# tobwei/APTAI

Measured on AMD Instinct MI355X. Metric: utterances/sec (10 s @ 16 kHz) train-step, higher is better.
Workload: dtype bf16

## Files before the change

### aptai_amd/_lib.py

```python
from __future__ import annotations

import ctypes
import os
import subprocess
import threading

import torch

_HERE = os.path.dirname(os.path.abspath(__file__))
CSRC = os.path.join(_HERE, "csrc")
LIB_PATH = os.environ.get("APTAI_HIP_LIB") or os.path.join(CSRC, "libaptai_hip.so")

_lib = None
_lock = threading.Lock()

_P, _I64, _I, _F, _U64 = ctypes.c_void_p, ctypes.c_int64, ctypes.c_int, ctypes.c_float, ctypes.c_uint64
ARGTYPES = {
    "aptai_layernorm_fwd": [_P, _P, _P, _P, _P, _P, _I64, _I64, _F, _I, _P],
    "aptai_layernorm_bwd": [_P, _P, _P, _P, _P, _P, _P, _P, _F, _U64, _P, _P, _P, _I64, _I64, _P, _P],
    "aptai_layernorm_bwd_workspace_bytes": [_I64, _I64],
    "aptai_layernorm_bwd_finalize_multi": [_P, _I64, _I64, _P],
    "aptai_layernorm_fwd_f32in": [_P, _P, _P, _P, _P, _I64, _I64, _F, _P],
    "aptai_layernorm_fwd_f32in_split": [_P, _P, _P, _P, _P, _I, _I64, _I64, _F, _P],
    "aptai_attention_fwd": [_P, _P, _P, _P, _P, _I64, _I64, _I64, _I64, _F, _F, _U64, _I, _P],
    "aptai_attention_bwd": [_P, _P, _P, _P, _P, _P, _P, _P, _I64, _I64, _I64, _I64, _F, _F, _U64, _I, _I, _P],
    "aptai_cast_f32_to_bf16": [_P, _P, _I64, _I64, _I64, _P],
    "aptai_conv_weight_to_bf16": [_P, _P, _I64, _I64, _I64, _P],
    "aptai_posconv_weight": [_P, _P, _P, _P, _P, _I64, _I64, _I64, _P],
    "aptai_posconv_pack": [_P, _P, _P, _P, _I64, _I64, _I64, _I64, _I64, _P],
    "aptai_frame_mask_fwd": [_P, _P, _P, _P, _I64, _I64, _I64, _I64, _P],
    "aptai_frame_mask_bwd": [_P, _P, _P, _P, _P, _I64, _I64, _I64, _I64, _P],
    "aptai_frame_mask_bwd_workspace_bytes": [_I64, _I64, _I64],
    "aptai_colsum_bf16": [_P, _I64, _P, _P, _I64, _I64, _I, _P],
    "aptai_colsum_workspace_bytes": [_I64, _I64],
    "aptai_dropout_bf16": [_P, _P, _I64, _F, _U64, _P],
    "aptai_dgelu_bf16": [_P, _P, _P, _I64, _P],
    "aptai_conv0_fwd": [_P, _I64, _I64, _P, _P, _P, _P, _I, _F, _P, _I64, _I64, _I64, _I64, _I64, _P, _P, _P],
    "aptai_conv0_bwd": [_P, _I64, _I64, _P, _P, _P, _P, _I, _F, _P, _I64, _I64, _P, _P, _P, _P, _P, _P, _P],
    "aptai_conv0_bwd_workspace_bytes": [_I64, _I64],
    "aptai_conv0_workspace_bytes": [_I64, _I64],
# ... 103 lines not shown
```

### aptai_amd/csrc/attention.hip

```cpp
#include "common.h"

namespace {

#ifdef APTAI_STAMPS
__device__ unsigned long long g_attn_stamps[3 * 1024 * 8];
#define ATTN_STAMP(k, slot)                                                                                       \
    do {                                                                                                          \
        if (threadIdx.x == 0) {                                                                                   \
            const int bl = blockIdx.x + gridDim.x * (blockIdx.y + gridDim.y * blockIdx.z);                        \
            if (bl < 1024) g_attn_stamps[((k) * 1024 + bl) * 8 + (slot)] = wall_clock64();                         \
        }                                                                                                         \
    } while (0)
#else
#define ATTN_STAMP(k, slot) do {} while (0)
#endif

constexpr int HD = 64;
constexpr float LOG2E = 1.4426950408889634f;

struct AttnArgs {
    const bf16_t* qkv; long ld;
    const int* lens;
    bf16_t* ctx; long ldo;
    float* lse2;
    float* o32;
    int B, Tp, H, heads;
    float c;
    float scale;
    uint32_t seed0, seed1, thr16; float dscale;
    const uint32_t* salt;
    const bf16_t* dctx;
    float* delta;
    bf16_t* dqkv;
    int skip_pad_q;
    int stagger;
    int xcd_remap;
    int q_prescaled;
};

__device__ __forceinline__ int tile_swz(int row) { return ((row >> 2) & 3) | (((row >> 1) & 1) << 2); }
__device__ __forceinline__ int tile_off(int row, int chunk) { return row * 128 + ((chunk ^ tile_swz(row)) << 4); }

struct LaneOffs {
    int rowk[4];
    int tr[2][2];
};
__device__ __forceinline__ LaneOffs lane_offs(int lane) {
    LaneOffs o;
    const int r31 = lane & 31, h = lane >> 5;
#pragma unroll
    for (int ds = 0; ds < 4; ++ds) o.rowk[ds] = tile_off(r31, 2 * ds + h);
    const int dgrp = (lane >> 4) & 1, i = lane & 15, qq = i >> 2, p = i & 3;
    const int trow = 4 * h + qq;
// ... 13 lines not shown
    return __builtin_bit_cast(bf16x8, r);
}

__device__ __forceinline__ bf16x8 pack8(const float* v) {
    u32x4 u = {pack2bf(v[0], v[1]), pack2bf(v[2], v[3]), pack2bf(v[4], v[5]), pack2bf(v[6], v[7])};
    return __builtin_bit_cast(bf16x8, u);
}

__device__ __forceinline__ int acc_row(int r, int h) { return (r & 3) + 8 * (r >> 2) + 4 * h; }

constexpr int OUT_PITCH = 144;
constexpr int STAGE_BYTES = 4 * 32 * OUT_PITCH;
constexpr int DQ_STAGE = 2 * 128 * 128;
constexpr int DKDV_BLOCKS = 3;
constexpr int DKDV_KV_BYTES = 2 * 128 * 128;

__device__ __forceinline__ void stage_rows128(char* dst, const bf16_t* src, long ld, int tid) {
#pragma unroll
    for (int it = 0; it < 4; ++it) {
        const int cid = it * 256 + tid, row = cid >> 3, ch = cid & 7;
        *(u32x4*)(dst + tile_off(row, ch)) = *(const u32x4*)(src + (long)row * ld + ch * 8);
    }
}
__device__ __forceinline__ void store_rows_bf16(char* sw, const f32x16 (&acc)[2], float scale, bf16_t* g_row0, long ld, int lane) {
    const int r31 = lane & 31, h = lane >> 5;
#pragma unroll
    for (int dt = 0; dt < 2; ++dt)
#pragma unroll
        for (int g4 = 0; g4 < 4; ++g4) {
            const int d = dt * 32 + 8 * g4 + 4 * h;
// ... 19 lines not shown
    int L = blockIdx.x + nt * (blockIdx.y + gridDim.y * blockIdx.z);
    if (a.xcd_remap && (total & 7) == 0) L = (L & 7) * (total >> 3) + (L >> 3);
    tile = L % nt;
    const int grp = L / nt;
    hd = grp % (int)gridDim.y;
    b = grp / (int)gridDim.y;
}

constexpr int FWD_BUF = 2 * 64 * 128;
constexpr int FWD_SMEM = 2 * FWD_BUF;
constexpr float REF_HEADROOM = 40.0f;
constexpr float REF_SUM_LIMIT = 1.4901161193847656e-08f;

template <bool V> struct Flag { static constexpr bool value = V; };

template <bool DROP>
__global__ __launch_bounds__(256, 3) void attn_fwd_kernel(AttnArgs a) {
    __shared__ __attribute__((aligned(16))) char smem[FWD_SMEM];
    ATTN_STAMP(0, 0);
    if (DROP) apply_salt(a.salt, a.seed0, a.seed1);
    const int tid = threadIdx.x, lane = tid & 63, wave = tid >> 6, h = lane >> 5;
    int tile_x, hd, b;
    attn_block(a, tile_x, hd, b);
    const int q0 = tile_x * 128 + wave * 32;
    int len = a.lens[b];
    len = len < 1 ? 1 : (len > a.Tp ? a.Tp : len);
    const int ntiles = (len + 63) >> 6;
    const long rowbase = (long)b * a.Tp;
    const int q = q0 + (lane & 31);
    const bf16_t* Qg = a.qkv + (rowbase + q) * a.ld + hd * HD;
    const bf16_t* Kg = a.qkv + rowbase * a.ld + a.H + hd * HD;
    const bf16_t* Vg = Kg + a.H;
// ... 11 lines not shown

    int soff[2];
    long goff[2];
#pragma unroll
    for (int it = 0; it < 2; ++it) {
        const int cid = it * 256 + tid, row = cid >> 3, ch = cid & 7;
        soff[it] = tile_off(row, ch);
        goff[it] = (long)row * a.ld + ch * 8;
    }
    u32x4 kreg[2], vreg[2];
    const long tile_stride = 64 * a.ld;
#pragma unroll
    for (int it = 0; it < 2; ++it) { kreg[it] = *(const u32x4*)(Kg + goff[it]); vreg[it] = *(const u32x4*)(Vg + goff[it]); }
    uint32_t hbase = 0;
    if (DROP) hbase = rng_hash((uint32_t)((b * a.heads + hd) * a.Tp + q), a.seed0, a.seed1) + (uint32_t)(2 * h) * ATTN_K1;
    const float c = a.c;
#pragma unroll
    for (int it = 0; it < 2; ++it) { *(u32x4*)(smem + soff[it]) = kreg[it]; *(u32x4*)(smem + 64 * 128 + soff[it]) = vreg[it]; }
    if (ntiles > 1) {
#pragma unroll
        for (int it = 0; it < 2; ++it) {
            kreg[it] = *(const u32x4*)(Kg + tile_stride + goff[it]);
            vreg[it] = *(const u32x4*)(Vg + tile_stride + goff[it]);
        }
    }
    __syncthreads();
    ATTN_STAMP(0, 1);

    auto tile = [&](auto first_flag, auto mask_flag, const int t) {
        constexpr bool FIRST = decltype(first_flag)::value, MASK = decltype(mask_flag)::value;
// ... 28 lines not shown
            for (int kt2 = 0; kt2 < 2; ++kt2)
#pragma unroll
                for (int r = 0; r < 16; ++r)
                    if (kbase + kt2 * 32 + acc_row(r, h) >= len) sT[kt2][r] = -INFINITY;
        }
        if (FIRST) {
            float mt = sT[0][0];
#pragma unroll
            for (int r = 1; r < 16; ++r) mt = fmaxf(mt, sT[0][r]);
#pragma unroll
            for (int r = 0; r < 16; ++r) mt = fmaxf(mt, sT[1][r]);
            mt = fmaxf(mt, __shfl_xor(mt, 32, 64));
            ref = fmaf(mt, c, REF_HEADROOM);
        }
        float psum = 0.f;
#pragma unroll
        for (int kt2 = 0; kt2 < 2; ++kt2) {
            bf16x8 vfr[2][2];
#pragma unroll
            for (int s = 0; s < 2; ++s)
#pragma unroll
                for (int dt = 0; dt < 2; ++dt) vfr[s][dt] = rd_tr(sV, lo, 2 * kt2 + s, dt);
            float x[16];
#pragma unroll
            for (int r = 0; r < 16; ++r) { x[r] = fast_exp2(fmaf(sT[kt2][r], c, -ref)); psum += x[r]; }
            if (DROP) {
#pragma unroll
                for (int r = 0; r < 16; r += 2) {
                    const uint32_t hsh = attn_mix(hbase + (uint32_t)(kbase / 2 + 16 * kt2 + acc_row(r, 0) / 2) * ATTN_K1);
                    x[r] = (hsh & 0xffffu) >= a.thr16 ? x[r] : 0.f;
                    x[r + 1] = (hsh >> 16) >= a.thr16 ? x[r + 1] : 0.f;
                }
            }
            const bf16x8 pf0 = pack8(&x[0]), pf1 = pack8(&x[8]);
#pragma unroll
            for (int dt = 0; dt < 2; ++dt) oT[dt] = __builtin_amdgcn_mfma_f32_32x32x16_bf16(vfr[0][dt], pf0, oT[dt], 0, 0, 0);
#pragma unroll
            for (int dt = 0; dt < 2; ++dt) oT[dt] = __builtin_amdgcn_mfma_f32_32x32x16_bf16(vfr[1][dt], pf1, oT[dt], 0, 0, 0);
        }
        psum += __shfl_xor(psum, 32, 64);
        l_run += psum;
        if (!FIRST && __builtin_amdgcn_ballot_w64(!(psum <= REF_SUM_LIMIT))) {
            if (!(psum <= REF_SUM_LIMIT)) {
                const float e = floorf(fast_log2(psum)) + REF_HEADROOM;
                const float sc = fast_exp2(-e);
                ref += e;
                l_run *= sc;
#pragma unroll
                for (int r = 0; r < 16; ++r) { oT[0][r] *= sc; oT[1][r] *= sc; }
            }
        }
        __syncthreads();
    };
    if (ntiles == 1) {
// ... 36 lines not shown
            __syncthreads();
#pragma unroll
            for (int i = 0; i < 4; ++i) {
                const int idx = i * 64 + lane, r = idx >> 3, ch = idx & 7;
                *(f32x4*)(a.o32 + orow + (long)r * a.ldo + dt * 32 + ch * 4) = *(const f32x4*)(sw + r * OUT_PITCH + ch * 16);
            }
        }
    }
    ATTN_STAMP(0, 3);
#ifdef APTAI_STAMPS
    asm volatile("s_waitcnt vmcnt(0)" ::: "memory");
    ATTN_STAMP(0, 4);
#endif
}

template <bool PRE>
__global__ __launch_bounds__(256, PRE ? DKDV_BLOCKS : 2) void attn_bwd_dkdv_kernel(AttnArgs a) {
    __shared__ __attribute__((aligned(16))) char smem[STAGE_BYTES + 384 + DKDV_KV_BYTES];
    char* sQ = smem;
    char* sD = smem + 32 * 128;
    float* sL = (float*)(smem + STAGE_BYTES);
    char* sKall = smem + STAGE_BYTES + 384;
    char* sVall = sKall + 128 * 128;
    ATTN_STAMP(1, 0);
    if (a.thr16) apply_salt(a.salt, a.seed0, a.seed1);
    const int tid = threadIdx.x, lane = tid & 63, wave = tid >> 6, h = lane >> 5;
    int tile_x, hd, b;
    attn_block(a, tile_x, hd, b);
    const int kb0 = tile_x * 128;
    const int key0 = kb0 + wave * 32;
    int len = a.lens[b];
    len = len < 1 ? 1 : (len > a.Tp ? a.Tp : len);
    const long rowbase = (long)b * a.Tp;
    const int key = key0 + (lane & 31);
    bf16_t* dK0 = a.dqkv + (rowbase + kb0) * a.ld + a.H + hd * HD;
    bf16_t* dV0 = dK0 + a.H;
    if (kb0 >= len) {
// ... 20 lines not shown
    const float* del = a.delta + ((long)b * a.heads + hd) * a.Tp;
    const int srow = tid >> 3, sch = tid & 7;
    const int soff = tile_off(srow, sch);
    const long gq = (long)srow * a.ld + sch * 8, gd = (long)srow * a.ldo + sch * 8;
    u32x4 qreg = *(const u32x4*)(Qb + gq), dreg = *(const u32x4*)(Db + gd);
    const float* stat = (tid < 8 ? lse : del) + (tid & 7) * 4;
    f32x4 sreg = (f32x4)(0.f);
    if (tid < 16) sreg = *(const f32x4*)stat;
    const bool key_ok = key < len;
    const bool wave_boundary = key0 + 32 > len;
    const uint32_t hshift = (key & 1) ? 16u : 0u;
    const float c = a.c;
    const uint32_t pairk = (uint32_t)(key >> 1) * ATTN_K1;
    const uint32_t rowid0 = (uint32_t)((b * a.heads + hd) * a.Tp) + (uint32_t)(tid & 31);
    uint32_t hreg = 0;
    if (a.thr16 && tid >= 32 && tid < 64) hreg = rng_hash(rowid0, a.seed0, a.seed1);
    ATTN_STAMP(1, 1);
    for (int t = 0; t < nq; ++t) {
        __syncthreads();
        *(u32x4*)(sQ + soff) = qreg;
        *(u32x4*)(sD + soff) = dreg;
        if (tid < 16) *(f32x4*)(sL + tid * 4) = PRE ? -sreg : sreg;
        if (a.thr16 && tid >= 32 && tid < 64) ((uint32_t*)sL)[64 + (tid & 31)] = hreg;
        __syncthreads();
        if (t + 1 < nq) {
            qreg = *(const u32x4*)(Qb + (long)(t + 1) * 32 * a.ld + gq);
            dreg = *(const u32x4*)(Db + (long)(t + 1) * 32 * a.ldo + gd);
            if (tid < 16) sreg = *(const f32x4*)(stat + (t + 1) * 32);
            if (a.thr16 && tid >= 32 && tid < 64) hreg = rng_hash(rowid0 + (uint32_t)((t + 1) * 32), a.seed0, a.seed1);
        }
        f32x16 cs = (f32x16)(0.f), cd = (f32x16)(0.f);
        if (PRE) {
#pragma unroll
            for (int g4 = 0; g4 < 4; ++g4) {
                const f32x4 l4 = *(const f32x4*)(sL + 8 * g4 + 4 * h);
                const f32x4 d4 = *(const f32x4*)(sL + 32 + 8 * g4 + 4 * h);
#pragma unroll
                for (int rr = 0; rr < 4; ++rr) { cs[4 * g4 + rr] = l4[rr]; cd[4 * g4 + rr] = d4[rr]; }
            }
        }
        f32x16 s = __builtin_amdgcn_mfma_f32_32x32x16_bf16(rd_row(sQ, lo, 0, 0), rd_row(sKall, lo, wave, 0), cs, 0, 0, 0);
        f32x16 dp = __builtin_amdgcn_mfma_f32_32x32x16_bf16(rd_row(sD, lo, 0, 0), rd_row(sVall, lo, wave, 0), cd, 0, 0, 0);
#pragma unroll
        for (int ds = 1; ds < 4; ++ds) {
// ... 11 lines not shown
                const f32x4 d4 = *(const f32x4*)(sL + 32 + 8 * g4 + 4 * h);
#pragma unroll
                for (int rr = 0; rr < 4; ++rr) {
                    pd[4 * g4 + rr] = fast_exp2(fmaf(s[4 * g4 + rr], c, -l4[rr]));
                    dsv[4 * g4 + rr] = d4[rr];
                }
            }
        }
        if (wave_boundary) {
#pragma unroll
            for (int r = 0; r < 16; ++r) pd[r] = key_ok ? pd[r] : 0.f;
        }
        if (a.thr16) {
#pragma unroll
            for (int g4 = 0; g4 < 4; ++g4) {
                const u32x4 rh = *(const u32x4*)((const uint32_t*)sL + 64 + 8 * g4 + 4 * h);
                f32x4 nd4 = (f32x4)(0.f);
                if (PRE) nd4 = *(const f32x4*)(sL + 32 + 8 * g4 + 4 * h);
#pragma unroll
                for (int rr = 0; rr < 4; ++rr) {
                    const int r = 4 * g4 + rr;
                    const uint32_t y = attn_mix(rh[rr] + pairk);
                    const bool k = ((y >> hshift) & 0xffffu) >= a.thr16;
                    const float p0 = pd[r];
                    if (PRE) dsv[r] = p0 * (k ? dp[r] : nd4[rr]);
                    else dsv[r] = p0 * ((k ? dp[r] : 0.f) - dsv[r]);
                    pd[r] = k ? p0 : 0.f;
                }
            }
        } else {
#pragma unroll
            for (int r = 0; r < 16; ++r) dsv[r] = PRE ? pd[r] * dp[r] : pd[r] * (dp[r] - dsv[r]);
        }
#pragma unroll
        for (int sstep = 0; sstep < 2; ++sstep) {
            const bf16x8 pf = pack8(&pd[8 * sstep]);
// ... 5 lines not shown
            }
        }
    }
    __syncthreads();
    ATTN_STAMP(1, 2);
    char* sw = smem + wave * (32 * OUT_PITCH);
    store_rows_bf16(sw, dKT, (PRE ? 0.6931471805599453f : a.scale) * a.dscale, dK0 + (long)(wave * 32) * a.ld, a.ld, lane);
    store_rows_bf16(sw, dVT, a.dscale, dV0 + (long)(wave * 32) * a.ld, a.ld, lane);
    ATTN_STAMP(1, 3);
#ifdef APTAI_STAMPS
    asm volatile("s_waitcnt vmcnt(0)" ::: "memory");
    ATTN_STAMP(1, 4);
#endif
}

template <bool PRE>
__global__ __launch_bounds__(256, 3) void attn_bwd_dq_kernel(AttnArgs a) {
    __shared__ __attribute__((aligned(16))) char smem[DQ_STAGE + 512];
    char* sK = smem;
    char* sV = smem + 32 * 128;
    float* sDel = (float*)(smem + DQ_STAGE);
    ATTN_STAMP(2, 0);
    if (a.thr16) apply_salt(a.salt, a.seed0, a.seed1);
    const int tid = threadIdx.x, lane = tid & 63, wave = tid >> 6, h = lane >> 5;
    int tile_x, hd, b;
    attn_block(a, tile_x, hd, b);
    const int qb0 = tile_x * 128;
    const int q = qb0 + wave * 32 + (lane & 31);
    int len = a.lens[b];
    len = len < 1 ? 1 : (len > a.Tp ? a.Tp : len);
    const long rowbase = (long)b * a.Tp;
// ... 53 lines not shown
        acc += __shfl_xor(acc, 4, 64);
        acc += __shfl_xor(acc, 2, 64);
        acc += __shfl_xor(acc, 1, 64);
        if (part == 0) sDel[row] = acc;
    }
    ATTN_STAMP(2, 7);
    __syncthreads();
    float del_q = sDel[wave * 32 + (lane & 31)];
    __syncthreads();
    del_q *= __frcp_rn(a.dscale);
    if (h == 0) a.delta[((long)b * a.heads + hd) * a.Tp + q] = del_q;
    f32x16 dQT[2];
    dQT[0] = dQT[1] = (f32x16)(0.f);
    const int nk = (len + 31) >> 5;
    uint32_t hbase = 0;
    if (a.thr16) hbase = rng_hash((uint32_t)((b * a.heads + hd) * a.Tp + q), a.seed0, a.seed1) + (uint32_t)(2 * h) * ATTN_K1;
    const float c = a.c;
    const f32x16 cs = (f32x16)(PRE ? -lse_q : 0.f), cd = (f32x16)(PRE ? -del_q : 0.f);
    ATTN_STAMP(2, 1);
    for (int t = 0; t < nk; ++t) {
        __syncthreads();
        *(u32x4*)(sK + soff) = kreg;
        *(u32x4*)(sV + soff) = vreg;
        __syncthreads();
        if (t + 1 < nk) {
            kreg = *(const u32x4*)(Kb + (long)(t + 1) * 32 * a.ld + gk);
            vreg = *(const u32x4*)(Vb + (long)(t + 1) * 32 * a.ld + gk);
        }
        f32x16 sT = __builtin_amdgcn_mfma_f32_32x32x16_bf16(rd_row(sK, lo, 0, 0), qf[0], cs, 0, 0, 0);
        f32x16 dpT = __builtin_amdgcn_mfma_f32_32x32x16_bf16(rd_row(sV, lo, 0, 0), df[0], cd, 0, 0, 0);
#pragma unroll
        for (int ds = 1; ds < 4; ++ds) {
            sT = __builtin_amdgcn_mfma_f32_32x32x16_bf16(rd_row(sK, lo, 0, ds), qf[ds], sT, 0, 0, 0);
            dpT = __builtin_amdgcn_mfma_f32_32x32x16_bf16(rd_row(sV, lo, 0, ds), df[ds], dpT, 0, 0, 0);
        }
        float dsv[16];
        const bool boundary = t * 32 + 32 > len;
#pragma unroll
        for (int r = 0; r < 16; ++r) {
            float p = PRE ? fast_exp2(sT[r]) : fast_exp2(fmaf(sT[r], c, -lse_q));
            if (boundary && (t * 32 + acc_row(r, h) >= len)) p = 0.f;
            dsv[r] = p;
        }
        if (a.thr16) {
            const float dropped = PRE ? -del_q : 0.f;
#pragma unroll
            for (int r = 0; r < 16; r += 2) {
                const uint32_t hsh = attn_mix(hbase + (uint32_t)(t * 16 + acc_row(r, 0) / 2) * ATTN_K1);
                dpT[r] = (hsh & 0xffffu) >= a.thr16 ? dpT[r] : dropped;
                dpT[r + 1] = (hsh >> 16) >= a.thr16 ? dpT[r + 1] : dropped;
            }
        }
#pragma unroll
        for (int r = 0; r < 16; ++r) dsv[r] *= PRE ? dpT[r] : (dpT[r] - del_q);
#pragma unroll
        for (int sstep = 0; sstep < 2; ++sstep) {
            const bf16x8 dsf = pack8(&dsv[8 * sstep]);
#pragma unroll
            for (int dt = 0; dt < 2; ++dt)
                dQT[dt] = __builtin_amdgcn_mfma_f32_32x32x16_bf16(rd_tr(sK, lo, sstep, dt), dsf, dQT[dt], 0, 0, 0);
        }
    }
    __syncthreads();
    ATTN_STAMP(2, 2);
    store_rows_bf16(smem + wave * (32 * OUT_PITCH), dQT, a.scale * a.dscale,
// ... 223 lines not shown
    static const int stagger = getenv("APTAI_ATTN_STAGGER") ? atoi(getenv("APTAI_ATTN_STAGGER")) : 0;
    a.stagger = stagger;
    static const int remap = getenv("APTAI_ATTN_XCD_REMAP") ? atoi(getenv("APTAI_ATTN_XCD_REMAP")) : 1;
    a.xcd_remap = remap;
    return APTAI_OK;
}

}

#ifdef APTAI_STAMPS
extern "C" int aptai_debug_read_attn_stamps(void* host_out) {
    return hipMemcpyFromSymbol(host_out, HIP_SYMBOL(g_attn_stamps), sizeof(g_attn_stamps)) == hipSuccess ? 0 : 1;
}
#endif

extern "C" int aptai_attention_fwd(const void* qkv, const int32_t* lens, void* ctx, float* lse2, float* ctx_f32, int64_t B,
                                   int64_t Tp, int64_t H, int64_t heads, float scale, float dropout_p, uint64_t seed,
                                   int q_prescaled, void* stream_) {
    AttnArgs a;
    int rc = fill_args(a, "aptai_attention_fwd", qkv, lens, B, Tp, H, heads, scale, dropout_p, seed, q_prescaled, stream_);
    if (rc) return rc;
    APTAI_REQUIRE(ctx != nullptr, "aptai_attention_fwd: null ctx");
    a.ctx = (bf16_t*)ctx; a.lse2 = lse2; a.o32 = ctx_f32;
    if (a.thr16) {
        APTAI_LAUNCH(attn_fwd_kernel<true>, dim3((unsigned)(Tp / 128), (unsigned)heads, (unsigned)B), dim3(256), 0,
                     (hipStream_t)stream_, a);
    } else {
        APTAI_LAUNCH(attn_fwd_kernel<false>, dim3((unsigned)(Tp / 128), (unsigned)heads, (unsigned)B), dim3(256), 0,
                     (hipStream_t)stream_, a);
    }
    APTAI_CHECK_LAUNCH("attn_fwd_kernel");
    return APTAI_OK;
}

extern "C" int aptai_attention_bwd(const void* qkv, const int32_t* lens, const void* ctx, const float* ctx_f32, const void* dctx,
                                   const float* lse2, float* delta_ws, void* dqkv, int64_t B, int64_t Tp, int64_t H,
                                   int64_t heads, float scale, float dropout_p, uint64_t seed, int dctx_zero_beyond_len,
                                   int q_prescaled, void* stream_) {
    hipStream_t stream = (hipStream_t)stream_;
    AttnArgs a;
    int rc = fill_args(a, "aptai_attention_bwd", qkv, lens, B, Tp, H, heads, scale, dropout_p, seed, q_prescaled, stream_);
    if (rc) return rc;
    APTAI_REQUIRE(ctx && dctx && lse2 && delta_ws && dqkv, "aptai_attention_bwd: null pointer");
    a.ctx = (bf16_t*)ctx; a.dctx = (const bf16_t*)dctx; a.lse2 = (float*)lse2; a.delta = delta_ws; a.o32 = (float*)ctx_f32; a.dqkv = (bf16_t*)dqkv;
    a.skip_pad_q = dctx_zero_beyond_len;
    dim3 grid((unsigned)(Tp / 128), (unsigned)heads, (unsigned)B);
    if (q_prescaled) {
        APTAI_LAUNCH(attn_bwd_dq_kernel<true>, grid, dim3(256), 0, stream, a);
        APTAI_CHECK_LAUNCH("attn_bwd_dq_kernel");
        APTAI_LAUNCH(attn_bwd_dkdv_kernel<true>, grid, dim3(256), 0, stream, a);
    } else {
        APTAI_LAUNCH(attn_bwd_dq_kernel<false>, grid, dim3(256), 0, stream, a);
        APTAI_CHECK_LAUNCH("attn_bwd_dq_kernel");
        APTAI_LAUNCH(attn_bwd_dkdv_kernel<false>, grid, dim3(256), 0, stream, a);
    }
    APTAI_CHECK_LAUNCH("attn_bwd_dkdv_kernel");
    return APTAI_OK;
}

extern "C" int aptai_attention_exact_fwd(const void* qkv_split, int64_t ld, const int32_t* lens, void* ctx_split, int64_t ldo, int64_t B,
                                         int64_t Tp, int64_t H, int64_t heads, int pieces, float scale, void* stream_) {
    APTAI_REQUIRE(qkv_split && lens && ctx_split, "aptai_attention_exact_fwd: null pointer");
    APTAI_REQUIRE(B > 0 && Tp > 0 && Tp % 128 == 0, "aptai_attention_exact_fwd: frames per utterance (%ld) must be a positive multiple of 128", (long)Tp);
    APTAI_REQUIRE(heads > 0 && H == heads * HD, "aptai_attention_exact_fwd: head_dim must be 64 (H=%ld heads=%ld)", (long)H, (long)heads);
    APTAI_REQUIRE(pieces == 3 || pieces == 6, "aptai_attention_exact_fwd: pieces must be 3 (f32x3) or 6 (f32x6)");
    APTAI_REQUIRE(ld >= 3 * pieces * H && ld % 8 == 0 && ldo >= pieces * H && ldo % 8 == 0, "aptai_attention_exact_fwd: row pitches (ld=%ld, ldo=%ld) too small "
                  "for %d slots of H=%ld or not a multiple of 8", (long)ld, (long)ldo, pieces, (long)H);
    APTAI_REQUIRE((uintptr_t)qkv_split % 16 == 0 && (uintptr_t)ctx_split % 16 == 0, "aptai_attention_exact_fwd: operands must be 16-byte aligned");
    AttnXArgs a;
    a.qkv = (const bf16_t*)qkv_split; a.ld = ld; a.lens = lens; a.ctx = (bf16_t*)ctx_split; a.ldo = ldo;
    a.B = (int)B; a.Tp = (int)Tp; a.H = (int)H; a.heads = (int)heads; a.slots = pieces;
    a.c = scale * LOG2E;
// ... 18 lines not shown
```

### aptai_amd/ops.py

```python
from __future__ import annotations

import ctypes
from typing import Optional

import torch

from . import _lib

EPI_BIAS, EPI_GELU, EPI_RESIDUAL, EPI_DROPOUT, EPI_DGELU, EPI_ALPHA, EPI_PRE_DGELU, EPI_MUL_AUX, EPI_RESIDUAL_F32, EPI_SPLIT_OUT, EPI_BIAS_ROW = 1, 2, 4, 8, 16, 32, 64, 128, 256, 512, 1024

c_void_p, c_i64, c_int, c_float, c_u64 = (ctypes.c_void_p, ctypes.c_int64, ctypes.c_int, ctypes.c_float,
                                          ctypes.c_uint64)


class GemmDesc(ctypes.Structure):
    _fields_ = [("A", c_void_p), ("lda", c_i64), ("B", c_void_p), ("ldb", c_i64), ("C", c_void_p), ("ldc", c_i64),
                ("M", c_i64), ("N", c_i64), ("K", c_i64),
                ("a_kmajor", c_int), ("b_kmajor", c_int), ("out_f32", c_int), ("flags", c_int),
                ("bias", c_void_p), ("residual", c_void_p), ("ldr", c_i64), ("out_pre", c_void_p),
                ("aux", c_void_p), ("ldaux", c_i64), ("alpha", c_float), ("dropout_p", c_float), ("seed", c_u64),
                ("split_k", c_int), ("accumulate", c_int), ("workspace", c_void_p), ("workspace_bytes", c_i64),
                ("batch_outer", c_int), ("batch_inner", c_int),
                ("batch_stride_a", c_i64 * 2), ("batch_stride_b", c_i64 * 2), ("batch_stride_c", c_i64 * 2),
                ("batch_stride_bias", c_i64 * 2), ("batch_stride_res", c_i64 * 2), ("batch_stride_aux", c_i64 * 2),
# ... 399 lines not shown


def layernorm_fwd_f32in_split(x32, gamma, beta, eps, pieces, *, want_f32=True):
    _dev(x32, gamma, beta)
    rows, cols = x32.shape
    y32 = torch.empty((rows, cols), device=x32.device, dtype=torch.float32) if want_f32 else None
    ys = torch.empty((rows, cols * pieces), device=x32.device, dtype=torch.bfloat16)
    _lib.call("aptai_layernorm_fwd_f32in_split", x32.data_ptr(), gamma.data_ptr(), beta.data_ptr(), _ptr(y32), ys.data_ptr(), pieces, rows, cols, eps, _stream())
    return y32, ys


def attention_qscale(H: int, heads: int) -> float:
    return (H // heads) ** -0.5 * ATTN_LOG2E


def attention_fwd(qkv, lens_i32, B, Tp, H, heads, *, dropout_p=0.0, seed=0, save_lse=True, q_prescaled=False):
    _dev(qkv, lens_i32)
    ctx = torch.empty((B * Tp, H), device=qkv.device, dtype=torch.bfloat16)
    lse2 = torch.empty((B, heads, Tp), device=qkv.device, dtype=torch.float32) if save_lse else None
    ctx32 = torch.empty((B * Tp, H), device=qkv.device, dtype=torch.float32) if save_lse else None
    _lib.call("aptai_attention_fwd", qkv.data_ptr(), lens_i32.data_ptr(), ctx.data_ptr(), _ptr(lse2), _ptr(ctx32), B, Tp, H,
              heads, (H // heads) ** -0.5, dropout_p, seed, int(q_prescaled), _stream())
    return ctx, (lse2, ctx32) if save_lse else None


def attention_bwd(qkv, lens_i32, ctx, dctx, stats, B, Tp, H, heads, *, dropout_p=0.0, seed=0, dctx_zero_beyond_len=False,
                  q_prescaled=False):
    lse2, ctx32 = stats
    _dev(qkv, lens_i32, ctx, dctx, lse2)
    dqkv = torch.empty_like(qkv)
    delta = torch.empty((B, heads, Tp), device=qkv.device, dtype=torch.float32)
    _lib.call("aptai_attention_bwd", qkv.data_ptr(), lens_i32.data_ptr(), ctx.data_ptr(), _ptr(ctx32), dctx.data_ptr(), lse2.data_ptr(),
              delta.data_ptr(), dqkv.data_ptr(), B, Tp, H, heads, (H // heads) ** -0.5, dropout_p, seed,
              int(dctx_zero_beyond_len), int(q_prescaled), _stream())
    return dqkv


def cast_bf16(src: torch.Tensor, dst: Optional[torch.Tensor] = None, ld_dst: Optional[int] = None) -> torch.Tensor:
    _dev(src, dst)
    src2 = src.reshape(src.shape[0], -1) if src.dim() > 1 else src.reshape(1, -1)
    rows, cols = src2.shape
    if dst is None:
        dst = torch.empty(src.shape, device=src.device, dtype=torch.bfloat16)
    _lib.call("aptai_cast_f32_to_bf16", src2.data_ptr(), dst.data_ptr(), rows, cols, ld_dst if ld_dst else cols, _stream())
    return dst


class CastPlan:

# ... 440 lines not shown
```

### aptai_amd/wav2vec2.py

```python
from __future__ import annotations

import json
import math
import os
from types import SimpleNamespace
from typing import List, Optional, Tuple

import numpy as np
import torch
import torch.nn as nn

from . import hostlogic, ops
from .config import W2V2Config


def _round_up(x: int, m: int) -> int:
    return (x + m - 1) // m * m


def _rows_with_zero_slack(rows: int, C: int, dev, slack: int = 8) -> torch.Tensor:
    t = torch.empty((rows, C), device=dev, dtype=torch.bfloat16)
    t[rows - slack:].zero_()
    return t

# ... 88 lines not shown
        p_a = cfg.activation_dropout if tr else 0.0
        p_att = cfg.attention_dropout if tr else 0.0
        s = SimpleNamespace(x=x)
        pre = cfg.do_stable_layer_norm
        mx = getattr(self, "mx", None)
        if mx is not None and not need:
            return self._fwd_mxfp8(x, params, mx)
        if pre:
            n1, s.m1, s.r1 = ops.layernorm_fwd(x, ln1w, ln1b, cfg.layer_norm_eps, save_stats=need)
            attn_in = n1
            s.n1 = n1
        else:
            attn_in = x
        s.qkv = ops.gemm(attn_in, w.wqkv, M, 3 * H, H, bias=w.bqkv, colscale=(H, ops.attention_qscale(H, cfg.num_attention_heads)))
        s.ctx, s.lse = ops.attention_fwd(s.qkv, self.lens, g.B, g.Tp, H, cfg.num_attention_heads, q_prescaled=True, dropout_p=p_att,
                                         seed=_seed(self.seed, 1), save_lse=need)
        s.s1 = ops.gemm(s.ctx, w.wo, M, H, H, bias=w.bo, residual=x, dropout_p=p_h, seed=_seed(self.seed, 2))
        if pre:
            ffn_in, s.m2, s.r2 = ops.layernorm_fwd(s.s1, ln2w, ln2b, cfg.layer_norm_eps, save_stats=need)
            s.n2 = ffn_in
        else:
            ffn_in, s.m1, s.r1 = ops.layernorm_fwd(s.s1, ln1w, ln1b, cfg.layer_norm_eps, save_stats=need)
            s.x1 = ffn_in
        s.u = torch.empty((M, I), device=x.device, dtype=torch.bfloat16) if need else None
        s.hact = ops.gemm(ffn_in, w.w1, M, I, H, bias=w.b1, gelu=True, out_pre=s.u, pre_dgelu=need and _PRE_DGELU, dropout_p=p_a,
                          seed=_seed(self.seed, 3))
        res2 = s.s1 if pre else ffn_in
        s.s2 = ops.gemm(s.hact, w.w2, M, H, I, bias=w.b2, residual=res2, dropout_p=p_h, seed=_seed(self.seed, 4))
        if pre:
            y = s.s2
        else:
# ... 132 lines not shown
        ones = ops.ones_kmajor(M, p.du.device)
        dw2, dw1, dwo, dwqkv, r2, r1, ro, rq = ops.gemm_grouped([
            (p.d_ffn_out, p.hact, H, I, M, tn), (p.du, p.ffn_in, I, H, M, tn), (p.d_att_out, p.ctx, H, H, M, tn),
            (p.dqkv, p.attn_in, 3 * H, H, M, tn),
            (ones, p.d_ffn_out, 8, H, M, tn), (ones, p.du, 8, I, M, tn), (ones, p.d_att_out, 8, H, M, tn),
            (ones, p.dqkv, 8, 3 * H, M, tn)])
        dbias2, dbias1, dbo, dbqkv = r2[0], r1[0], ro[0], rq[0]
        return (dwqkv[0:H], dwqkv[H:2 * H], dwqkv[2 * H:3 * H], dbqkv[0:H], dbqkv[H:2 * H], dbqkv[2 * H:3 * H], dwo, dbo, dw1, dbias1,
                dw2, dbias2)


_SIDE_STREAMS = {}
_GROUPED_WGRAD = os.environ.get("APTAI_GROUPED_WGRAD", "1") != "0"
_PRE_DGELU = os.environ.get("APTAI_PRE_DGELU", "1") != "0"
_SPEC_ON_DEVICE = os.environ.get("APTAI_SPEC_ON_DEVICE", "1") != "0"
_USE_SIDE_STREAM = os.environ.get("APTAI_SIDE_STREAM", "0") != "0"


def _side_stream(device):
    st = _SIDE_STREAMS.get(device)
    if st is None:
        st = torch.cuda.Stream(device=device)
        _SIDE_STREAMS[device] = st
    return st


class _FrontImpl:

    def __init__(self, cfg, geom, lens_i32, spec, training, seed, model):
        self.cfg, self.g, self.lens, self.spec, self.training, self.seed, self.model = cfg, geom, lens_i32, spec, training, seed, model
# ... 712 lines not shown
```

### include/aptai_hip.h

```cpp
#ifndef APTAI_HIP_H
#define APTAI_HIP_H
#include <stdint.h>

#ifdef __cplusplus
extern "C" {
#endif

typedef enum {
    APTAI_OK = 0,
    APTAI_ERR_INVALID = -1,
    APTAI_ERR_LAUNCH = -2,
    APTAI_ERR_NO_DEVICE = -3
} aptai_status;

const char* aptai_last_error(void);
int aptai_version(void);
int aptai_device_check(char* name, int name_len);
int aptai_set_seed_salt(void* stream, const void* device_ptr_2xu32);
int aptai_set_frame_bounds(void* stream, const void* device_ptr_2xi32);

enum {
    APTAI_EPI_BIAS = 1,
    APTAI_EPI_GELU = 2,
    APTAI_EPI_RESIDUAL = 4,
// ... 62 lines not shown
                              int64_t cols, float eps, void* stream);
int aptai_layernorm_fwd_f32in_split(const float* x, const float* gamma, const float* beta, float* y_f32, void* y_split, int pieces,
                                    int64_t rows, int64_t cols, float eps, void* stream);
int aptai_layernorm_bwd(const void* dy, const void* x, const float* mean, const float* rstd, const float* gamma,
                        const void* dres, void* dx, void* dx_drop, float dropout_p, uint64_t seed, float* dgamma,
                        float* dbeta, void* workspace, int64_t rows, int64_t cols, const float* beta_if_gelu_after,
                        void* stream);
int64_t aptai_layernorm_bwd_workspace_bytes(int64_t rows, int64_t cols);
int aptai_layernorm_bwd_finalize_multi(const int64_t* table_dev, int64_t njobs, int64_t max_cols, void* stream);

int aptai_attention_fwd(const void* qkv, const int32_t* lens, void* ctx, float* lse2, float* ctx_f32, int64_t B, int64_t Tp,
                        int64_t H, int64_t heads, float scale, float dropout_p, uint64_t seed, int q_prescaled, void* stream);
int aptai_attention_bwd(const void* qkv, const int32_t* lens, const void* ctx, const float* ctx_f32, const void* dctx,
                        const float* lse2, float* delta_ws, void* dqkv, int64_t B, int64_t Tp, int64_t H, int64_t heads, float scale,
                        float dropout_p, uint64_t seed, int dctx_zero_beyond_len, int q_prescaled, void* stream);

int aptai_cast_f32_to_bf16(const float* src, void* dst, int64_t rows, int64_t cols, int64_t ld_dst, void* stream);
int aptai_cast_multi(const int64_t* table_dev, int64_t njobs, int64_t max_n, void* stream);
int aptai_adam_multi(const int64_t* table_dev, const int64_t* dyn_dev, int64_t njobs, int64_t max_n, float lr, float beta1,
                     float beta2, float eps, float weight_decay, void* stream);
int aptai_conv_weight_to_bf16(const float* src, void* dst, int64_t N, int64_t C, int64_t Kw, void* stream);
int aptai_posconv_weight(const float* v, const float* gain, float* norm_ws, void* w_fwd, void* w_dgrad, int64_t H,
                         int64_t groups, int64_t Kw, void* stream);
int aptai_posconv_weight_bwd(const float* dw_fwd, const float* v, const float* gain, const float* norm, float* dv, float* dgain,
                             float* workspace, int64_t H, int64_t groups, int64_t Kw, void* stream);
int aptai_posconv_gemm(const void* xg, int64_t first_row, const void* w, const float* bias, const void* residual, void* out,
                       void* out_pre, int64_t B, int64_t Tp, int64_t H, int64_t groups, int64_t Kw, int64_t pad, int gelu,
                       void* stream);
int aptai_posconv_wgrad(const void* du_g, const void* x_g, float* dw, int64_t B, int64_t Tp, int64_t H, int64_t groups, int64_t Kw,
                        int64_t pad, void* stream);
// ... 105 lines not shown
```

Before: 1758.

## Store attention dropout keep-mask bitmask in forward, reuse in backward kernels

The attention forward kernel now packs the per-element dropout keep decisions into a 1-bit-per-element mask in global memory using ballot/addc bit shifting. Both backward kernels (dQ and dK/dV) read this mask instead of recomputing the hash-based RNG for every score element. This trades hash ALU work in backward for extra global writes and reads of the mask (B*heads*Tp*Tp/8 bytes) and some extra register and shared memory use. It is enabled by default through an environment flag.

```diff
diff --git a/aptai_amd/_lib.py b/aptai_amd/_lib.py
--- a/aptai_amd/_lib.py
+++ b/aptai_amd/_lib.py
@@ -24,6 +24,8 @@
     "aptai_layernorm_fwd_f32in_split": [_P, _P, _P, _P, _P, _I, _I64, _I64, _F, _P],
     "aptai_attention_fwd": [_P, _P, _P, _P, _P, _I64, _I64, _I64, _I64, _F, _F, _U64, _I, _P],
     "aptai_attention_bwd": [_P, _P, _P, _P, _P, _P, _P, _P, _I64, _I64, _I64, _I64, _F, _F, _U64, _I, _I, _P],
+    "aptai_attention_fwd_keep": [_P, _P, _P, _P, _P, _I64, _I64, _I64, _I64, _F, _F, _U64, _I, _P, _P],
+    "aptai_attention_bwd_keep": [_P, _P, _P, _P, _P, _P, _P, _P, _I64, _I64, _I64, _I64, _F, _F, _U64, _I, _I, _P, _P],
     "aptai_cast_f32_to_bf16": [_P, _P, _I64, _I64, _I64, _P],
     "aptai_conv_weight_to_bf16": [_P, _P, _I64, _I64, _I64, _P],
     "aptai_posconv_weight": [_P, _P, _P, _P, _P, _I64, _I64, _I64, _P],
diff --git a/aptai_amd/csrc/attention.hip b/aptai_amd/csrc/attention.hip
--- a/aptai_amd/csrc/attention.hip
+++ b/aptai_amd/csrc/attention.hip
@@ -1,4 +1,6 @@
 #include "common.h"
+
+#include <utility>
 
 namespace {
 
@@ -36,7 +38,31 @@
     int stagger;
     int xcd_remap;
     int q_prescaled;
+    uint32_t* keep;
 };
+
+__device__ __forceinline__ long keep_word(int bh, int Tp, int qg, int kt) { return (((long)bh * (Tp >> 5) + qg) * (Tp >> 6) + kt) * 64; }
+__host__ __device__ constexpr int keep_bit(int kt2, int r) { return 31 - 16 * kt2 - r; }
+__device__ __forceinline__ uint32_t keep_shift_in(uint32_t bits, bool k) {
+    uint32_t r;
+    uint64_t carry;
+    asm("v_addc_co_u32_e64 %0, %1, %2, %2, %3" : "=v"(r), "=s"(carry) : "v"(bits), "s"(__builtin_amdgcn_ballot_w64(k)));
+    return r;
+}
+template <int N, class F, int... I> __device__ __forceinline__ void static_for(F&& f, std::integer_sequence<int, I...>) {
+    (f(std::integral_constant<int, I>{}), ...);
+}
+template <int N, class F> __device__ __forceinline__ void static_for(F&& f) { static_for<N>(f, std::make_integer_sequence<int, N>{}); }
+template <int POS> __device__ __forceinline__ uint32_t keep_ones(uint32_t w) {
+    uint32_t m;
+    asm("v_bfe_i32 %0, %1, %2, 1" : "=v"(m) : "v"(w), "i"(POS));
+    return m;
+}
+__device__ __forceinline__ void keep_select(uint32_t w, uint32_t pos, float p, float x, float y, float& p_keep, float& sel) {
+    uint32_t m;
+    asm("v_bfe_i32 %2, %3, %4, 1\n\tv_bfi_b32 %1, %2, %5, %6\n\tv_and_b32 %0, %2, %7"
+        : "=&v"(p_keep), "=&v"(sel), "=&v"(m) : "v"(w), "v"(pos), "v"(x), "v"(y), "v"(p));
+}
 
 __device__ __forceinline__ int tile_swz(int row) { return ((row >> 2) & 3) | (((row >> 1) & 1) << 2); }
 __device__ __forceinline__ int tile_off(int row, int chunk) { return row * 128 + ((chunk ^ tile_swz(row)) << 4); }
@@ -80,6 +106,7 @@
 constexpr int DQ_STAGE = 2 * 128 * 128;
 constexpr int DKDV_BLOCKS = 3;
 constexpr int DKDV_KV_BYTES = 2 * 128 * 128;
+constexpr int DKDV_STAT_BYTES = 192 * 4;
 
 __device__ __forceinline__ void stage_rows128(char* dst, const bf16_t* src, long ld, int tid) {
 #pragma unroll
@@ -129,8 +156,9 @@
 
 template <bool V> struct Flag { static constexpr bool value = V; };
 
-template <bool DROP>
+template <bool DROP, bool KEEP>
 __global__ __launch_bounds__(256, 3) void attn_fwd_kernel(AttnArgs a) {
+    static_assert(DROP || !KEEP, "the keep mask exists only with dropout");
     __shared__ __attribute__((aligned(16))) char smem[FWD_SMEM];
     ATTN_STAMP(0, 0);
     if (DROP) apply_salt(a.salt, a.seed0, a.seed1);
@@ -172,6 +200,8 @@
     for (int it = 0; it < 2; ++it) { kreg[it] = *(const u32x4*)(Kg + goff[it]); vreg[it] = *(const u32x4*)(Vg + goff[it]); }
     uint32_t hbase = 0;
     if (DROP) hbase = rng_hash((uint32_t)((b * a.heads + hd) * a.Tp + q), a.seed0, a.seed1) + (uint32_t)(2 * h) * ATTN_K1;
+    uint32_t* keep_dst = nullptr;
+    if (KEEP) keep_dst = a.keep + keep_word(b * a.heads + hd, a.Tp, q0 >> 5, 0) + lane;
     const float c = a.c;
 #pragma unroll
     for (int it = 0; it < 2; ++it) { *(u32x4*)(smem + soff[it]) = kreg[it]; *(u32x4*)(smem + 64 * 128 + soff[it]) = vreg[it]; }
@@ -230,6 +260,7 @@
             ref = fmaf(mt, c, REF_HEADROOM);
         }
         float psum = 0.f;
+        uint32_t kbits = 0;
 #pragma unroll
         for (int kt2 = 0; kt2 < 2; ++kt2) {
             bf16x8 vfr[2][2];
@@ -244,8 +275,13 @@
 #pragma unroll
                 for (int r = 0; r < 16; r += 2) {
                     const uint32_t hsh = attn_mix(hbase + (uint32_t)(kbase / 2 + 16 * kt2 + acc_row(r, 0) / 2) * ATTN_K1);
-                    x[r] = (hsh & 0xffffu) >= a.thr16 ? x[r] : 0.f;
-                    x[r + 1] = (hsh >> 16) >= a.thr16 ? x[r + 1] : 0.f;
+                    const bool k0 = (hsh & 0xffffu) >= a.thr16, k1 = (hsh >> 16) >= a.thr16;
+                    x[r] = k0 ? x[r] : 0.f;
+                    x[r + 1] = k1 ? x[r + 1] : 0.f;
+                    if (KEEP) {
+                        kbits = keep_shift_in(kbits, k0);
+                        kbits = keep_shift_in(kbits, k1);
+                    }
                 }
             }
             const bf16x8 pf0 = pack8(&x[0]), pf1 = pack8(&x[8]);
@@ -254,6 +290,7 @@
 #pragma unroll
             for (int dt = 0; dt < 2; ++dt) oT[dt] = __builtin_amdgcn_mfma_f32_32x32x16_bf16(vfr[1][dt], pf1, oT[dt], 0, 0, 0);
         }
+        if (KEEP) keep_dst[(long)t * 64] = kbits;
         psum += __shfl_xor(psum, 32, 64);
         l_run += psum;
         if (!FIRST && __builtin_amdgcn_ballot_w64(!(psum <= REF_SUM_LIMIT))) {
@@ -320,13 +357,13 @@
 #endif
 }
 
-template <bool PRE>
+template <bool PRE, bool KEEP>
 __global__ __launch_bounds__(256, PRE ? DKDV_BLOCKS : 2) void attn_bwd_dkdv_kernel(AttnArgs a) {
-    __shared__ __attribute__((aligned(16))) char smem[STAGE_BYTES + 384 + DKDV_KV_BYTES];
+    __shared__ __attribute__((aligned(16))) char smem[STAGE_BYTES + DKDV_STAT_BYTES + DKDV_KV_BYTES];
     char* sQ = smem;
     char* sD = smem + 32 * 128;
     float* sL = (float*)(smem + STAGE_BYTES);
-    char* sKall = smem + STAGE_BYTES + 384;
+    char* sKall = smem + STAGE_BYTES + DKDV_STAT_BYTES;
     char* sVall = sKall + 128 * 128;
     ATTN_STAMP(1, 0);
     if (a.thr16) apply_salt(a.salt, a.seed0, a.seed1);
@@ -377,20 +414,30 @@
     const uint32_t pairk = (uint32_t)(key >> 1) * ATTN_K1;
     const uint32_t rowid0 = (uint32_t)((b * a.heads + hd) * a.Tp) + (uint32_t)(tid & 31);
     uint32_t hreg = 0;
-    if (a.thr16 && tid >= 32 && tid < 64) hreg = rng_hash(rowid0, a.seed0, a.seed1);
+    if (!KEEP && a.thr16 && tid >= 32 && tid < 64) hreg = rng_hash(rowid0, a.seed0, a.seed1);
+    const uint32_t* keep_src = nullptr;
+    uint32_t mreg = 0;
+    const bool keep_ld = KEEP && tid < 128 && kb0 + 64 * (tid >> 6) < len;
+    if (KEEP) keep_src = a.keep + keep_word(b * a.heads + hd, a.Tp, 0, kb0 >> 6);
+    if (keep_ld) mreg = keep_src[(uint32_t)tid];
+    const int ko = lane & 31, hf = (ko >> 2) & 1, rk = (ko & 3) | ((ko >> 3) << 2);
+    const int kbit = keep_bit(wave & 1, rk);
+    const uint32_t* sKeep = (const uint32_t*)sL + 64 + (wave >> 1) * 64 + hf * 32 + 4 * h;
     ATTN_STAMP(1, 1);
     for (int t = 0; t < nq; ++t) {
         __syncthreads();
         *(u32x4*)(sQ + soff) = qreg;
         *(u32x4*)(sD + soff) = dreg;
         if (tid < 16) *(f32x4*)(sL + tid * 4) = PRE ? -sreg : sreg;
-        if (a.thr16 && tid >= 32 && tid < 64) ((uint32_t*)sL)[64 + (tid & 31)] = hreg;
+        if (!KEEP && a.thr16 && tid >= 32 && tid < 64) ((uint32_t*)sL)[64 + (tid & 31)] = hreg;
+        if (KEEP && tid < 128) ((uint32_t*)sL)[64 + tid] = mreg;
         __syncthreads();
         if (t + 1 < nq) {
             qreg = *(const u32x4*)(Qb + (long)(t + 1) * 32 * a.ld + gq);
             dreg = *(const u32x4*)(Db + (long)(t + 1) * 32 * a.ldo + gd);
             if (tid < 16) sreg = *(const f32x4*)(stat + (t + 1) * 32);
-            if (a.thr16 && tid >= 32 && tid < 64) hreg = rng_hash(rowid0 + (uint32_t)((t + 1) * 32), a.seed0, a.seed1);
+            if (!KEEP && a.thr16 && tid >= 32 && tid < 64) hreg = rng_hash(rowid0 + (uint32_t)((t + 1) * 32), a.seed0, a.seed1);
+            if (keep_ld) mreg = (keep_src + (long)(t + 1) * a.Tp)[(uint32_t)tid];
         }
         f32x16 cs = (f32x16)(0.f), cd = (f32x16)(0.f);
         if (PRE) {
@@ -432,12 +479,20 @@
         if (a.thr16) {
 #pragma unroll
             for (int g4 = 0; g4 < 4; ++g4) {
-                const u32x4 rh = *(const u32x4*)((const uint32_t*)sL + 64 + 8 * g4 + 4 * h);
+                const u32x4 rh = KEEP ? *(const u32x4*)(sKeep + 8 * g4) : *(const u32x4*)((const uint32_t*)sL + 64 + 8 * g4 + 4 * h);
                 f32x4 nd4 = (f32x4)(0.f);
                 if (PRE) nd4 = *(const f32x4*)(sL + 32 + 8 * g4 + 4 * h);
 #pragma unroll
                 for (int rr = 0; rr < 4; ++rr) {
                     const int r = 4 * g4 + rr;
+                    if (KEEP) {
+                        const float p0 = pd[r];
+                        float sel;
+                        keep_select(rh[rr], kbit, p0, dp[r], PRE ? nd4[rr] : 0.f, pd[r], sel);
+                        dsv[r] = PRE ? p0 * sel : p0 * (sel - dsv[r]);
+                        if (rr & 1) __builtin_amdgcn_sched_barrier(0);
+                        continue;
+                    }
                     const uint32_t y = attn_mix(rh[rr] + pairk);
                     const bool k = ((y >> hshift) & 0xffffu) >= a.thr16;
                     const float p0 = pd[r];
@@ -473,7 +528,7 @@
 #endif
 }
 
-template <bool PRE>
+template <bool PRE, bool KEEP>
 __global__ __launch_bounds__(256, 3) void attn_bwd_dq_kernel(AttnArgs a) {
     __shared__ __attribute__((aligned(16))) char smem[DQ_STAGE + 512];
     char* sK = smem;
@@ -557,7 +612,13 @@
     dQT[0] = dQT[1] = (f32x16)(0.f);
     const int nk = (len + 31) >> 5;
     uint32_t hbase = 0;
-    if (a.thr16) hbase = rng_hash((uint32_t)((b * a.heads + hd) * a.Tp + q), a.seed0, a.seed1) + (uint32_t)(2 * h) * ATTN_K1;
+    if (!KEEP && a.thr16) hbase = rng_hash((uint32_t)((b * a.heads + hd) * a.Tp + q), a.seed0, a.seed1) + (uint32_t)(2 * h) * ATTN_K1;
+    const uint32_t* keep_src = nullptr;
+    uint32_t mcur = 0;
+    if (KEEP) {
+        keep_src = a.keep + keep_word(b * a.heads + hd, a.Tp, (qb0 >> 5) + wave, 0) + lane;
+        mcur = keep_src[0];
+    }
     const float c = a.c;
     const f32x16 cs = (f32x16)(PRE ? -lse_q : 0.f), cd = (f32x16)(PRE ? -del_q : 0.f);
     ATTN_STAMP(2, 1);
@@ -566,9 +627,11 @@
         *(u32x4*)(sK + soff) = kreg;
         *(u32x4*)(sV + soff) = vreg;
         __syncthreads();
+        const uint32_t mw = mcur << ((t & 1) << 4);
         if (t + 1 < nk) {
             kreg = *(const u32x4*)(Kb + (long)(t + 1) * 32 * a.ld + gk);
             vreg = *(const u32x4*)(Vb + (long)(t + 1) * 32 * a.ld + gk);
+            if (KEEP && (t & 1)) mcur = keep_src[(long)((t + 1) >> 1) * 64];
         }
         f32x16 sT = __builtin_amdgcn_mfma_f32_32x32x16_bf16(rd_row(sK, lo, 0, 0), qf[0], cs, 0, 0, 0);
         f32x16 dpT = __builtin_amdgcn_mfma_f32_32x32x16_bf16(rd_row(sV, lo, 0, 0), df[0], cd, 0, 0, 0);
@@ -587,11 +650,19 @@
         }
         if (a.thr16) {
             const float dropped = PRE ? -del_q : 0.f;
-#pragma unroll
-            for (int r = 0; r < 16; r += 2) {
-                const uint32_t hsh = attn_mix(hbase + (uint32_t)(t * 16 + acc_row(r, 0) / 2) * ATTN_K1);
-                dpT[r] = (hsh & 0xffffu) >= a.thr16 ? dpT[r] : dropped;
-                dpT[r + 1] = (hsh >> 16) >= a.thr16 ? dpT[r + 1] : dropped;
+            if (KEEP) {
+                static_for<16>([&](auto rc) {
+                    constexpr int r = decltype(rc)::value;
+                    const uint32_t m = keep_ones<keep_bit(0, r)>(mw);
+                    dpT[r] = __uint_as_float((__float_as_uint(dpT[r]) & m) | (__float_as_uint(dropped) & ~m));
+                });
+            } else {
+#pragma unroll
+                for (int r = 0; r < 16; r += 2) {
+                    const uint32_t hsh = attn_mix(hbase + (uint32_t)(t * 16 + acc_row(r, 0) / 2) * ATTN_K1);
+                    dpT[r] = (hsh & 0xffffu) >= a.thr16 ? dpT[r] : dropped;
+                    dpT[r + 1] = (hsh >> 16) >= a.thr16 ? dpT[r + 1] : dropped;
+                }
             }
         }
 #pragma unroll
@@ -845,48 +916,69 @@
 }
 #endif
 
-extern "C" int aptai_attention_fwd(const void* qkv, const int32_t* lens, void* ctx, float* lse2, float* ctx_f32, int64_t B,
-                                   int64_t Tp, int64_t H, int64_t heads, float scale, float dropout_p, uint64_t seed,
-                                   int q_prescaled, void* stream_) {
+extern "C" int aptai_attention_fwd_keep(const void* qkv, const int32_t* lens, void* ctx, float* lse2, float* ctx_f32, int64_t B,
+                                        int64_t Tp, int64_t H, int64_t heads, float scale, float dropout_p, uint64_t seed,
+                                        int q_prescaled, uint32_t* keep, void* stream_) {
     AttnArgs a;
     int rc = fill_args(a, "aptai_attention_fwd", qkv, lens, B, Tp, H, heads, scale, dropout_p, seed, q_prescaled, stream_);
     if (rc) return rc;
     APTAI_REQUIRE(ctx != nullptr, "aptai_attention_fwd: null ctx");
-    a.ctx = (bf16_t*)ctx; a.lse2 = lse2; a.o32 = ctx_f32;
-    if (a.thr16) {
-        APTAI_LAUNCH(attn_fwd_kernel<true>, dim3((unsigned)(Tp / 128), (unsigned)heads, (unsigned)B), dim3(256), 0,
-                     (hipStream_t)stream_, a);
+    APTAI_REQUIRE((uintptr_t)keep % 4 == 0, "aptai_attention_fwd_keep: keep must be 4-byte aligned");
+    a.ctx = (bf16_t*)ctx; a.lse2 = lse2; a.o32 = ctx_f32; a.keep = keep;
+    const dim3 grid((unsigned)(Tp / 128), (unsigned)heads, (unsigned)B);
+    if (a.thr16 && keep) {
+        APTAI_LAUNCH((attn_fwd_kernel<true, true>), grid, dim3(256), 0, (hipStream_t)stream_, a);
+    } else if (a.thr16) {
+        APTAI_LAUNCH((attn_fwd_kernel<true, false>), grid, dim3(256), 0, (hipStream_t)stream_, a);
     } else {
-        APTAI_LAUNCH(attn_fwd_kernel<false>, dim3((unsigned)(Tp / 128), (unsigned)heads, (unsigned)B), dim3(256), 0,
-                     (hipStream_t)stream_, a);
+        APTAI_LAUNCH((attn_fwd_kernel<false, false>), grid, dim3(256), 0, (hipStream_t)stream_, a);
     }
     APTAI_CHECK_LAUNCH("attn_fwd_kernel");
     return APTAI_OK;
 }
 
-extern "C" int aptai_attention_bwd(const void* qkv, const int32_t* lens, const void* ctx, const float* ctx_f32, const void* dctx,
-                                   const float* lse2, float* delta_ws, void* dqkv, int64_t B, int64_t Tp, int64_t H,
-                                   int64_t heads, float scale, float dropout_p, uint64_t seed, int dctx_zero_beyond_len,
+extern "C" int aptai_attention_fwd(const void* qkv, const int32_t* lens, void* ctx, float* lse2, float* ctx_f32, int64_t B,
+                                   int64_t Tp, int64_t H, int64_t heads, float scale, float dropout_p, uint64_t seed,
                                    int q_prescaled, void* stream_) {
+    return aptai_attention_fwd_keep(qkv, lens, ctx, lse2, ctx_f32, B, Tp, H, heads, scale, dropout_p, seed, q_prescaled, nullptr, stream_);
+}
+
+namespace {
+template <bool PRE, bool KEEP>
+int launch_bwd(const AttnArgs& a, dim3 grid, hipStream_t stream) {
+    APTAI_LAUNCH((attn_bwd_dq_kernel<PRE, KEEP>), grid, dim3(256), 0, stream, a);
+    APTAI_CHECK_LAUNCH("attn_bwd_dq_kernel");
+    APTAI_LAUNCH((attn_bwd_dkdv_kernel<PRE, KEEP>), grid, dim3(256), 0, stream, a);
+    APTAI_CHECK_LAUNCH("attn_bwd_dkdv_kernel");
+    return APTAI_OK;
+}
+}
+
+extern "C" int aptai_attention_bwd_keep(const void* qkv, const int32_t* lens, const void* ctx, const float* ctx_f32, const void* dctx,
+                                        const float* lse2, float* delta_ws, void* dqkv, int64_t B, int64_t Tp, int64_t H,
+                                        int64_t heads, float scale, float dropout_p, uint64_t seed, int dctx_zero_beyond_len,
+                                        int q_prescaled, const uint32_t* keep, void* stream_) {
     hipStream_t stream = (hipStream_t)stream_;
     AttnArgs a;
     int rc = fill_args(a, "aptai_attention_bwd", qkv, lens, B, Tp, H, heads, scale, dropout_p, seed, q_prescaled, stream_);
     if (rc) return rc;
     APTAI_REQUIRE(ctx && dctx && lse2 && delta_ws && dqkv, "aptai_attention_bwd: null pointer");
+    APTAI_REQUIRE((uintptr_t)keep % 4 == 0, "aptai_attention_bwd_keep: keep must be 4-byte aligned");
     a.ctx = (bf16_t*)ctx; a.dctx = (const bf16_t*)dctx; a.lse2 = (float*)lse2; a.delta = delta_ws; a.o32 = (float*)ctx_f32; a.dqkv = (bf16_t*)dqkv;
     a.skip_pad_q = dctx_zero_beyond_len;
-    dim3 grid((unsigned)(Tp / 128), (unsigned)heads, (unsigned)B);
-    if (q_prescaled) {
-        APTAI_LAUNCH(attn_bwd_dq_kernel<true>, grid, dim3(256), 0, stream, a);
-        APTAI_CHECK_LAUNCH("attn_bwd_dq_kernel");
-        APTAI_LAUNCH(attn_bwd_dkdv_kernel<true>, grid, dim3(256), 0, stream, a);
-    } else {
-        APTAI_LAUNCH(attn_bwd_dq_kernel<false>, grid, dim3(256), 0, stream, a);
-        APTAI_CHECK_LAUNCH("attn_bwd_dq_kernel");
-        APTAI_LAUNCH(attn_bwd_dkdv_kernel<false>, grid, dim3(256), 0, stream, a);
-    }
-    APTAI_CHECK_LAUNCH("attn_bwd_dkdv_kernel");
-    return APTAI_OK;
+    a.keep = (uint32_t*)keep;
+    const dim3 grid((unsigned)(Tp / 128), (unsigned)heads, (unsigned)B);
+    const bool use_keep = a.thr16 && keep;
+    if (q_prescaled) return use_keep ? launch_bwd<true, true>(a, grid, stream) : launch_bwd<true, false>(a, grid, stream);
+    return use_keep ? launch_bwd<false, true>(a, grid, stream) : launch_bwd<false, false>(a, grid, stream);
+}
+
+extern "C" int aptai_attention_bwd(const void* qkv, const int32_t* lens, const void* ctx, const float* ctx_f32, const void* dctx,
+                                   const float* lse2, float* delta_ws, void* dqkv, int64_t B, int64_t Tp, int64_t H,
+                                   int64_t heads, float scale, float dropout_p, uint64_t seed, int dctx_zero_beyond_len,
+                                   int q_prescaled, void* stream_) {
+    return aptai_attention_bwd_keep(qkv, lens, ctx, ctx_f32, dctx, lse2, delta_ws, dqkv, B, Tp, H, heads, scale, dropout_p, seed,
+                                    dctx_zero_beyond_len, q_prescaled, nullptr, stream_);
 }
 
 extern "C" int aptai_attention_exact_fwd(const void* qkv_split, int64_t ld, const int32_t* lens, void* ctx_split, int64_t ldo, int64_t B,
diff --git a/aptai_amd/ops.py b/aptai_amd/ops.py
--- a/aptai_amd/ops.py
+++ b/aptai_amd/ops.py
@@ -437,25 +437,38 @@
     return (H // heads) ** -0.5 * ATTN_LOG2E
 
 
-def attention_fwd(qkv, lens_i32, B, Tp, H, heads, *, dropout_p=0.0, seed=0, save_lse=True, q_prescaled=False):
+def attention_keep_shape(B, Tp, heads):
+    return (B, heads, Tp // 32, Tp // 64, 64)
+
+
+def attention_fwd(qkv, lens_i32, B, Tp, H, heads, *, dropout_p=0.0, seed=0, save_lse=True, q_prescaled=False, save_keep=False):
     _dev(qkv, lens_i32)
     ctx = torch.empty((B * Tp, H), device=qkv.device, dtype=torch.bfloat16)
     lse2 = torch.empty((B, heads, Tp), device=qkv.device, dtype=torch.float32) if save_lse else None
     ctx32 = torch.empty((B * Tp, H), device=qkv.device, dtype=torch.float32) if save_lse else None
-    _lib.call("aptai_attention_fwd", qkv.data_ptr(), lens_i32.data_ptr(), ctx.data_ptr(), _ptr(lse2), _ptr(ctx32), B, Tp, H,
-              heads, (H // heads) ** -0.5, dropout_p, seed, int(q_prescaled), _stream())
-    return ctx, (lse2, ctx32) if save_lse else None
+    keep = None
+    if save_lse and save_keep and dropout_p > 0:
+        keep = torch.empty(attention_keep_shape(B, Tp, heads), device=qkv.device, dtype=torch.int32)
+    _lib.call("aptai_attention_fwd_keep", qkv.data_ptr(), lens_i32.data_ptr(), ctx.data_ptr(), _ptr(lse2), _ptr(ctx32), B, Tp, H,
+              heads, (H // heads) ** -0.5, dropout_p, seed, int(q_prescaled), _ptr(keep), _stream())
+    if not save_lse:
+        return ctx, None
+    return ctx, (lse2, ctx32) if keep is None else (lse2, ctx32, keep)
 
 
 def attention_bwd(qkv, lens_i32, ctx, dctx, stats, B, Tp, H, heads, *, dropout_p=0.0, seed=0, dctx_zero_beyond_len=False,
                   q_prescaled=False):
-    lse2, ctx32 = stats
+    lse2, ctx32 = stats[0], stats[1]
+    keep = stats[2] if len(stats) > 2 else None
     _dev(qkv, lens_i32, ctx, dctx, lse2)
+    if keep is not None and (tuple(keep.shape) != attention_keep_shape(B, Tp, heads) or keep.dtype != torch.int32):
+        raise _lib.AptaiHipError(f"attention_bwd: keep mask {tuple(keep.shape)} {keep.dtype}, expected "
+                                 f"{attention_keep_shape(B, Tp, heads)} int32")
     dqkv = torch.empty_like(qkv)
     delta = torch.empty((B, heads, Tp), device=qkv.device, dtype=torch.float32)
-    _lib.call("aptai_attention_bwd", qkv.data_ptr(), lens_i32.data_ptr(), ctx.data_ptr(), _ptr(ctx32), dctx.data_ptr(), lse2.data_ptr(),
+    _lib.call("aptai_attention_bwd_keep", qkv.data_ptr(), lens_i32.data_ptr(), ctx.data_ptr(), _ptr(ctx32), dctx.data_ptr(), lse2.data_ptr(),
               delta.data_ptr(), dqkv.data_ptr(), B, Tp, H, heads, (H // heads) ** -0.5, dropout_p, seed,
-              int(dctx_zero_beyond_len), int(q_prescaled), _stream())
+              int(dctx_zero_beyond_len), int(q_prescaled), _ptr(keep), _stream())
     return dqkv
 
 
diff --git a/aptai_amd/wav2vec2.py b/aptai_amd/wav2vec2.py
--- a/aptai_amd/wav2vec2.py
+++ b/aptai_amd/wav2vec2.py
@@ -126,7 +126,7 @@
             attn_in = x
         s.qkv = ops.gemm(attn_in, w.wqkv, M, 3 * H, H, bias=w.bqkv, colscale=(H, ops.attention_qscale(H, cfg.num_attention_heads)))
         s.ctx, s.lse = ops.attention_fwd(s.qkv, self.lens, g.B, g.Tp, H, cfg.num_attention_heads, q_prescaled=True, dropout_p=p_att,
-                                         seed=_seed(self.seed, 1), save_lse=need)
+                                         seed=_seed(self.seed, 1), save_lse=need, save_keep=_ATTN_KEEP_MASK)
         s.s1 = ops.gemm(s.ctx, w.wo, M, H, H, bias=w.bo, residual=x, dropout_p=p_h, seed=_seed(self.seed, 2))
         if pre:
             ffn_in, s.m2, s.r2 = ops.layernorm_fwd(s.s1, ln2w, ln2b, cfg.layer_norm_eps, save_stats=need)
@@ -289,6 +289,7 @@
 _GROUPED_WGRAD = os.environ.get("APTAI_GROUPED_WGRAD", "1") != "0"
 _PRE_DGELU = os.environ.get("APTAI_PRE_DGELU", "1") != "0"
 _SPEC_ON_DEVICE = os.environ.get("APTAI_SPEC_ON_DEVICE", "1") != "0"
+_ATTN_KEEP_MASK = os.environ.get("APTAI_ATTN_MASK", "1") != "0"
 _USE_SIDE_STREAM = os.environ.get("APTAI_SIDE_STREAM", "0") != "0"
 
 
diff --git a/include/aptai_hip.h b/include/aptai_hip.h
--- a/include/aptai_hip.h
+++ b/include/aptai_hip.h
@@ -100,6 +100,13 @@
 int aptai_attention_bwd(const void* qkv, const int32_t* lens, const void* ctx, const float* ctx_f32, const void* dctx,
                         const float* lse2, float* delta_ws, void* dqkv, int64_t B, int64_t Tp, int64_t H, int64_t heads, float scale,
                         float dropout_p, uint64_t seed, int dctx_zero_beyond_len, int q_prescaled, void* stream);
+int aptai_attention_fwd_keep(const void* qkv, const int32_t* lens, void* ctx, float* lse2, float* ctx_f32, int64_t B, int64_t Tp,
+                             int64_t H, int64_t heads, float scale, float dropout_p, uint64_t seed, int q_prescaled, uint32_t* keep,
+                             void* stream);
+int aptai_attention_bwd_keep(const void* qkv, const int32_t* lens, const void* ctx, const float* ctx_f32, const void* dctx,
+                             const float* lse2, float* delta_ws, void* dqkv, int64_t B, int64_t Tp, int64_t H, int64_t heads, float scale,
+                             float dropout_p, uint64_t seed, int dctx_zero_beyond_len, int q_prescaled, const uint32_t* keep,
+                             void* stream);
 
 int aptai_cast_f32_to_bf16(const float* src, void* dst, int64_t rows, int64_t cols, int64_t ld_dst, void* stream);
 int aptai_cast_multi(const int64_t* table_dev, int64_t njobs, int64_t max_n, void* stream);
```

Result: no change. 1748, median of 2 (-0.6%).
